# buaacyw/MeshAnything

Hardware: NVIDIA H100
Metric: face-tokens/sec (350M, 800-face cap) (higher is better)
Workload: dtype f16 weights/activations, f32 accumulate

## Files before the change

meshanything_b200/csrc/api.cu:

```cuda
#include <stdarg.h>
#include <stdlib.h>
#include <stdio.h>
#include <string.h>

#include <atomic>
#include <map>
#include <mutex>
#include <vector>

#include "canon.cuh"
#include "internal.h"

namespace ma {

static thread_local char g_err[512] = "";
static std::atomic<unsigned long long> g_launches{0};

void set_error(const char* fmt, ...) {
  va_list ap;
  va_start(ap, fmt);
  vsnprintf(g_err, sizeof(g_err), fmt, ap);
  va_end(ap);
}
void count_launch(int n) { g_launches += (unsigned long long)n; }
// ... 303 lines not shown
  if (!logits || !out_tokens || B < 1 || vocab < 1) {
    set_error("ma_sample_tokens: bad arguments");
    return 1;
  }
  SampleArgs sa;
  memset(&sa, 0, sizeof(sa));
  sa.logits = (const __half*)logits; sa.vocab = vocab; sa.B = B; sa.max_new = 1; sa.eos_id = -1; sa.pad_id = -1;
  sa.do_sample = sampling ? sampling->do_sample : 0;
  sa.top_k = sampling ? sampling->top_k : 0;
  sa.top_p = sampling ? sampling->top_p : 1.0f;
  sa.seed = sampling ? sampling->seed : 0;
  sa.first = 1; sa.token_out = out_tokens; sa.support_out = out_support;
  return launch_sample(sa, (cudaStream_t)stream);
}

size_t ma_kv_cache_bytes(int n_layers, int B, int tmax) {
  return (size_t)n_layers * 2 * B * NHEAD * (size_t)tmax * HD * sizeof(__half);
}

size_t ma_decoder_workspace_bytes(int B, int tmax) { return carve(nullptr, B, tmax, 8195 + 61).total; }

int ma_decode_generate(const ma_decoder_weights* w, const float* prefix, int B, int tmax, int max_new,
                       const ma_sampling* sampling, int eos_id, int pad_id, void* kv, void* ws_, int32_t* out_ids,
                       int32_t* out_lens, const int32_t* forced_ids, void* logits_out, int flags, void* stream) {
  if (!w || !prefix || !kv || !ws_ || !out_ids || B <= 0 || max_new <= 0) {
    set_error("ma_decode_generate: bad arguments");
    return 1;
  }
  if (check_decode_args("ma_decode_generate", w, B, tmax, max_new)) return 1;
  std::lock_guard<std::mutex> lock(g_mu);
  if (ensure_globals()) return 1;
  cudaStream_t user = (cudaStream_t)stream;
  cudaStream_t st = g_stream;
  cudaEventRecord(g_ev_in, user);
  cudaStreamWaitEvent(st, g_ev_in, 0);

  const long T = tmax;
  DecWs ws = carve(ws_, B, tmax, 8195 + 61);
  cudaMemsetAsync(ws.attn_scratch, 0, ws.attn_scratch_bytes, st);
  cudaMemsetAsync(ws.attn_scratch_pre, 0, ws.attn_scratch_pre_bytes, st);
  cudaMemsetAsync(ws.fast, 0, fast_workspace_bytes(), st);
  if (launch_fill_i32(out_ids, pad_id, (long)B * max_new, st)) return 1;

  SampleArgs sa;
  fill_sample_args(sa, w, ws, B, max_new, sampling, eos_id, pad_id, out_ids);
  sa.first = 1; sa.forced = forced_ids; sa.logits_out = (__half*)logits_out;
  sa.all_done = ws.all_done;

  const bool tc = use_tc(B, sa.do_sample, flags);
  if (tc) cudaMemsetAsync(ws.tc_scratch, 0, linear_ws_scratch_bytes(), st);
  const bool fast = (B == 1) && !(flags & MA_GEN_NO_FAST);
  bool mega = fast && !sa.do_sample && !(flags & MA_GEN_NO_MEGA) && mega_fits(tmax) && mega_supported();
  if (fast) sa.nkeys_next = fast_nkeys_ptr(ws.fast);
  if (mega && mega_prepare(w, ws.mega, st)) mega = false;

  for (int b0 = 0; b0 < B; b0 += PREFILL_SEQS) {
    const int nb = std::min(PREFILL_SEQS, B - b0), M = nb * PREFIX;
    if (launch_embed_prefix(w, prefix + (size_t)b0 * PREFIX * HID, nb, ws.hres, ws.x16, ws.nkeys, st)) return 1;
    if (run_layers(w, ws, kv, B, T, M, PREFIX, b0, PREFIX, st, tc)) return 1;
    if (launch_gather_rows(ws.x16, HID, PREFIX - 1, PREFIX, nb, ws.lastx16 + (size_t)b0 * HID, st)) return 1;
  }
  if (dec_linear(tc, ws, w->lm_head, nullptr, ws.lastx16, HID, ws.logits, w->vocab, B, w->vocab, HID, MA_EPI_NONE, st))
    return 1;
  if (launch_sample(sa, st)) return 1;
  sa.first = 0;
  sa.nkeys_next = nullptr;


  const bool use_graph = !(flags & MA_GEN_NO_GRAPH);
  const bool early = !(flags & MA_GEN_NO_EARLY_EXIT) && !forced_ids;
  const int CHECK_EVERY = 64;
  const unsigned long long whash = use_graph ? weights_hash(w) : 0;
  bool flag_pending = false;
  int rc = 0;
  if (mega) {
    const int MEGA_STEPS = 512;
    for (int i = 1; i < max_new && rc == 0; i += MEGA_STEPS) {
      rc = mega_enqueue(w, ws.s, tmax, (__half*)kv, ws.mega, sa, std::min(MEGA_STEPS, max_new - i), i - 1,
                        (flags & MA_GEN_TRACE) ? 1 : 0, st);
    }
  }
  for (int i = 1; i < max_new && rc == 0 && !mega; i++) {
    const int ctx = PREFIX + i;
    const int bucket = fast ? 0 : (ctx + 1023) / 1024;
    const int max_keys = fast ? tmax : std::min(tmax, bucket * 1024);
    auto enqueue = [&](cudaStream_t s) -> int {
      if (fast) return fast_step_enqueue(w, ws.s, tmax, (__half*)kv, ws.fast, sa, !(flags & MA_GEN_NO_PDL), s);
      return enqueue_batched_step(w, ws, kv, B, T, max_keys, sa, s, tc);
    };
    if (!use_graph) {
      rc = enqueue(st);
    } else {
      GraphKey key;
      memset(&key, 0, sizeof(key));
      key.w = w; key.kv = kv; key.ws = ws_; key.out_ids = out_ids; key.forced = forced_ids; key.logits_out = logits_out;
      key.B = B; key.tmax = tmax; key.max_new = max_new; key.bucket = bucket; key.flags = flags;
      key.do_sample = sa.do_sample; key.top_k = sa.top_k; key.eos = eos_id; key.pad = pad_id; key.top_p = sa.top_p;
      key.seed = sa.do_sample ? sa.seed : 0;
      key.whash = whash;
      key.ws_mode = linear_ws_mode();
      if (launch_cached_graph(key, st, enqueue)) return 1;
    }
    if (early && (i % CHECK_EVERY) == 0) {
      if (flag_pending && cudaEventQuery(g_ev_flag) == cudaSuccess) {
        if (*g_flag_host == 1) break;
        flag_pending = false;
      }
      if (!flag_pending) {
        cudaMemcpyAsync(g_flag_host, ws.all_done, sizeof(int), cudaMemcpyDeviceToHost, st);
        cudaEventRecord(g_ev_flag, st);
        flag_pending = true;
      }
    }
  }
  if (rc) return rc;
  if (out_lens) cudaMemcpyAsync(out_lens, ws.s.lens, sizeof(int) * B, cudaMemcpyDeviceToDevice, st);
  cudaEventRecord(g_ev_out, st);
  cudaStreamWaitEvent(user, g_ev_out, 0);
  return check_launch("ma_decode_generate") ? 0 : 1;
}



static int slots_enter(void* stream, cudaStream_t* st) {
  if (ensure_globals()) return 1;
  cudaEventRecord(g_ev_in, (cudaStream_t)stream);
  cudaStreamWaitEvent(g_stream, g_ev_in, 0);
  *st = g_stream;
  return 0;
}
static int slots_leave(void* stream, const char* who) {
  cudaEventRecord(g_ev_out, g_stream);
  cudaStreamWaitEvent((cudaStream_t)stream, g_ev_out, 0);
  return check_launch(who) ? 0 : 1;
}

int ma_decode_slots_init(int B, int tmax, int pad_id, void* ws_, void* stream) {
  if (!ws_ || B <= 0 || tmax < PREFIX + 1) {
    set_error("ma_decode_slots_init: bad arguments");
    return 1;
  }
  std::lock_guard<std::mutex> lock(g_mu);
  cudaStream_t st;
  if (slots_enter(stream, &st)) return 1;
  DecWs ws = carve(ws_, B, tmax, 8195 + 61);
  cudaMemsetAsync(ws.attn_scratch, 0, ws.attn_scratch_bytes, st);
  cudaMemsetAsync(ws.attn_scratch_pre, 0, ws.attn_scratch_pre_bytes, st);
  cudaMemsetAsync(ws.tc_scratch, 0, linear_ws_scratch_bytes(), st);
  if (launch_fill_i32(ws.s.pos, PREFIX, B, st) || launch_fill_i32(ws.s.gen, 0, B, st) ||
      launch_fill_i32(ws.s.tok, pad_id, B, st) || launch_fill_i32(ws.s.finished, 1, B, st) ||
      launch_fill_i32(ws.s.lens, 0, B, st) || launch_fill_i32(ws.s.sid, 0, B, st)) return 1;
  return slots_leave(stream, "ma_decode_slots_init");
}

int ma_decode_slot_stream(int slot, int B, int tmax, int stream_id, void* ws_, void* stream) {
  if (!ws_ || slot < 0 || slot >= B) {
    set_error("ma_decode_slot_stream: bad arguments (slot %d of %d)", slot, B);
    return 1;
  }
  std::lock_guard<std::mutex> lock(g_mu);
  cudaStream_t st;
  if (slots_enter(stream, &st)) return 1;
  DecWs ws = carve(ws_, B, tmax, 8195 + 61);
  if (launch_fill_i32(ws.s.sid + slot, stream_id, 1, st)) return 1;
  return slots_leave(stream, "ma_decode_slot_stream");
}

int ma_decode_slots_seek(int B, int tmax, int pos, int gen, int tok, void* ws_, void* stream) {
  if (!ws_ || B <= 0 || pos < PREFIX || pos >= tmax || gen < 1) {
    set_error("ma_decode_slots_seek: bad arguments (pos %d of tmax %d)", pos, tmax);
// ... 117 lines not shown
```

meshanything_b200/csrc/attention.cu:

```cuda
#include "canon.cuh"
#include "internal.h"

namespace ma {

constexpr int ATT_THREADS = 256;
constexpr int PART = 66;

struct AttnSmem {
  __half k[MA_ATTN_CHUNK * HD];
  __half v[MA_ATTN_CHUNK * HD];
  float s[MA_ATTN_CHUNK];
  float red[8][65];
  float wmax[8];
  uint64_t bar[2];
  int last;
};

struct AttnArgs {
  const __half* q;
  int ldq;
  const __half* K;
  const __half* V;
  long T;
  int H;
  int rows_per_slot;
  const int* slots;
  const int* nkeys;
  float scale;
  __half* out;
  int ldo;
  float* part;
  int* counters;
  int max_chunks;
  int decode_prefetch;
};

__global__ void __launch_bounds__(ATT_THREADS) attention_kernel(AttnArgs a) {
  extern __shared__ __align__(128) unsigned char smem_raw[];
  AttnSmem& sm = *reinterpret_cast<AttnSmem*>(smem_raw);
  const int c = blockIdx.x, h = blockIdx.y, m = blockIdx.z;
  const int tid = threadIdx.x, warp = tid >> 5, lane = tid & 31, grp = lane >> 3, li = lane & 7;

  if (!a.decode_prefetch) pdl_wait();
  const int n = min(a.nkeys[m], a.max_chunks * MA_ATTN_CHUNK);
  if (c * MA_ATTN_CHUNK >= n) return;
  const int len = min(MA_ATTN_CHUNK, n - c * MA_ATTN_CHUNK);
  const int nch = (n + MA_ATTN_CHUNK - 1) / MA_ATTN_CHUNK;
  const int slot = a.slots ? a.slots[m] : m / a.rows_per_slot;
  const long base = (((long)slot * a.H + h) * a.T + (long)c * MA_ATTN_CHUNK) * HD;

  const int len_early = a.decode_prefetch ? max(0, min(len, (n - 1) - c * MA_ATTN_CHUNK)) : 0;
  if (tid == 0) {
    mbar_init(&sm.bar[0], 1);
    mbar_init(&sm.bar[1], 1);
    mbar_fence_init();
    if (len_early > 0) {
      mbar_expect_tx(&sm.bar[0], 2u * len_early * HD * 2);
      bulk_g2s(sm.k, a.K + base, len_early * HD * 2, &sm.bar[0]);
      bulk_g2s(sm.v, a.V + base, len_early * HD * 2, &sm.bar[0]);
    }
  }
  if (a.decode_prefetch) pdl_wait();
  pdl_trigger();
  if (tid == 0) {
    const int rest = len - len_early;
    if (rest > 0) {
      mbar_expect_tx(&sm.bar[1], 2u * rest * HD * 2);
      bulk_g2s(sm.k + len_early * HD, a.K + base + (long)len_early * HD, rest * HD * 2, &sm.bar[1]);
      bulk_g2s(sm.v + len_early * HD, a.V + base + (long)len_early * HD, rest * HD * 2, &sm.bar[1]);
    }
  }
  float qf[8];
  {
    uint4 u = *reinterpret_cast<const uint4*>(a.q + (long)m * a.ldq + h * HD + 8 * li);
    unpack8(u, qf);
  }
  __syncthreads();
  if (len_early > 0) mbar_wait(&sm.bar[0], 0);
  if (len - len_early > 0) mbar_wait(&sm.bar[1], 0);

  float lmax = -INFINITY;
#pragma unroll
  for (int rho = 0; rho < MA_ATTN_CHUNK / 32; rho++) {
    const int r = 32 * rho + 4 * warp + grp;
    const int rr = min(r, len - 1);
    uint4 u = *reinterpret_cast<const uint4*>(sm.k + rr * HD + 8 * li);
    float kf[8];
    unpack8(u, kf);
    float p = 0.0f;
#pragma unroll
    for (int j = 0; j < 8; j++) p = ffma(qf[j], kf[j], p);
    p = fadd(p, __shfl_xor_sync(0xffffffffu, p, 4));
    p = fadd(p, __shfl_xor_sync(0xffffffffu, p, 2));
    p = fadd(p, __shfl_xor_sync(0xffffffffu, p, 1));
    const float s = fmul(p, a.scale);
    if (r < len) {
      if (li == 0) sm.s[r] = s;
      lmax = fmaxf(lmax, s);
    }
  }
  lmax = warp_max(lmax);
  if (lane == 0) sm.wmax[warp] = lmax;
  __syncthreads();
  float cmax = sm.wmax[0];
#pragma unroll
  for (int w = 1; w < 8; w++) cmax = fmaxf(cmax, sm.wmax[w]);

  float l = 0.0f, o[8];
#pragma unroll
  for (int j = 0; j < 8; j++) o[j] = 0.0f;
#pragma unroll
  for (int rho = 0; rho < MA_ATTN_CHUNK / 32; rho++) {
    const int r = 32 * rho + 4 * warp + grp;
    if (r < len) {
      const float e = ma_exp(fsub(sm.s[r], cmax));
      l = fadd(l, e);
      uint4 u = *reinterpret_cast<const uint4*>(sm.v + r * HD + 8 * li);
      const float pf = __half2float(__float2half_rn(e));
      float vf[8];
      unpack8(u, vf);
#pragma unroll
      for (int j = 0; j < 8; j++) o[j] = ffma(pf, vf[j], o[j]);
    }
  }
  l = fadd(l, __shfl_xor_sync(0xffffffffu, l, 16));
  l = fadd(l, __shfl_xor_sync(0xffffffffu, l, 8));
#pragma unroll
  for (int j = 0; j < 8; j++) {
    o[j] = fadd(o[j], __shfl_xor_sync(0xffffffffu, o[j], 16));
    o[j] = fadd(o[j], __shfl_xor_sync(0xffffffffu, o[j], 8));
  }
  if (grp == 0) {
#pragma unroll
    for (int j = 0; j < 8; j++) sm.red[warp][8 * li + j] = o[j];
    if (li == 0) sm.red[warp][64] = l;
  }
  __syncthreads();
  float* part = a.part + (((long)m * a.H + h) * a.max_chunks) * PART;
  if (tid < 65) {
    float x[8];
#pragma unroll
    for (int w = 0; w < 8; w++) x[w] = sm.red[w][tid];
    const float r = fadd(fadd(fadd(x[0], x[1]), fadd(x[2], x[3])), fadd(fadd(x[4], x[5]), fadd(x[6], x[7])));
    if (nch == 1) {
      sm.red[0][tid] = r;
    } else {
      part[c * PART + (tid < 64 ? tid : 65)] = r;
      if (tid == 64) part[c * PART + 64] = cmax;
    }
  }
  if (nch > 1) {
    __threadfence();
    __syncthreads();
    if (tid == 0) {
      int* cnt = a.counters + (long)m * a.H + h;
      const int prev = atomicAdd(cnt, 1);
      sm.last = (prev == nch - 1);
      if (sm.last) *cnt = 0;
    }
    __syncthreads();
    if (!sm.last) return;
    __threadfence();
    if (tid < 64) {
      float M = -INFINITY;
      for (int cc = 0; cc < nch; cc++) M = fmaxf(M, __ldcg(part + cc * PART + 64));
      float L = 0.0f, O = 0.0f;
      for (int cc = 0; cc < nch; cc++) {
        const float w = ma_exp(fsub(__ldcg(part + cc * PART + 64), M));
        L = ffma(__ldcg(part + cc * PART + 65), w, L);
        O = ffma(__ldcg(part + cc * PART + tid), w, O);
      }
      a.out[(long)m * a.ldo + h * HD + tid] = __float2half_rn(__fdiv_rn(O, L));
    }
  } else {
    __syncthreads();
    if (tid < 64) {
      const float L = sm.red[0][64], O = sm.red[0][tid];
      a.out[(long)m * a.ldo + h * HD + tid] = __float2half_rn(__fdiv_rn(O, L));
    }
  }
}

size_t attention_scratch_bytes(int M, int H, int max_keys) {
  const size_t chunks = (size_t)(max_keys + MA_ATTN_CHUNK - 1) / MA_ATTN_CHUNK;
  return (size_t)M * H * chunks * PART * sizeof(float) + (size_t)M * H * sizeof(int) + 256;
}

int launch_attention_ex(const __half* q, int ldq, const __half* K, const __half* V, long T, int H, int rows_per_slot,
                        const int* slots, const int* nkeys, int max_keys, int M, float scale, __half* out, int ldo,
                        void* scratch, int decode_prefetch, bool pdl, cudaStream_t st) {
  if (M <= 0) return 0;
  static bool attr_done = false;
  if (!attr_done) {
    cudaFuncSetAttribute(attention_kernel, cudaFuncAttributeMaxDynamicSharedMemorySize, (int)sizeof(AttnSmem));
    attr_done = true;
  }
  const int chunks = (max_keys + MA_ATTN_CHUNK - 1) / MA_ATTN_CHUNK;
  AttnArgs a;
  a.q = q; a.ldq = ldq; a.K = K; a.V = V; a.T = T; a.H = H;
  a.rows_per_slot = rows_per_slot > 0 ? rows_per_slot : 1;
  a.slots = slots; a.nkeys = nkeys; a.scale = scale; a.out = out; a.ldo = ldo;
  a.counters = reinterpret_cast<int*>(scratch);
  size_t coff = ((size_t)M * H * sizeof(int) + 255) & ~(size_t)255;
  a.part = reinterpret_cast<float*>(reinterpret_cast<char*>(scratch) + coff);
  a.max_chunks = chunks;
  a.decode_prefetch = decode_prefetch;
  dim3 grid(chunks, H, M);
  cudaLaunchConfig_t cfg = {};
  cfg.gridDim = grid;
  cfg.blockDim = dim3(ATT_THREADS);
  cfg.dynamicSmemBytes = sizeof(AttnSmem);
  cfg.stream = st;
  cudaLaunchAttribute at[1];
  at[0].id = cudaLaunchAttributeProgrammaticStreamSerialization;
  at[0].val.programmaticStreamSerializationAllowed = 1;
  cfg.attrs = at;
  cfg.numAttrs = pdl ? 1 : 0;
  cudaLaunchKernelEx(&cfg, attention_kernel, a);
  count_launch();
  return check_launch("attention_kernel") ? 0 : 1;
}

int launch_attention(const __half* q, int ldq, const __half* K, const __half* V, long T, int H, int rows_per_slot,
                     const int* slots, const int* nkeys, int max_keys, int M, float scale, __half* out, int ldo,
                     void* scratch, cudaStream_t st) {
  return launch_attention_ex(q, ldq, K, V, T, H, rows_per_slot, slots, nkeys, max_keys, M, scale, out, ldo, scratch, 0,
                             false, st);
}

}
```

meshanything_b200/csrc/canon.cuh:

```cuda
#pragma once
#include <cuda_fp16.h>
#include <cuda_runtime.h>
#include <stdint.h>

#include "../../include/ma_canon_constants.h"

namespace ma {

__device__ __forceinline__ float fadd(float a, float b) { return __fadd_rn(a, b); }
__device__ __forceinline__ float fsub(float a, float b) { return __fsub_rn(a, b); }
__device__ __forceinline__ float fmul(float a, float b) { return __fmul_rn(a, b); }
__device__ __forceinline__ float ffma(float a, float b, float c) { return __fmaf_rn(a, b, c); }

__device__ __forceinline__ float ma_exp(float x) {
  if (x < MA_EXP_FLUSH) return 0.0f;
  float y = fmul(x, MA_LOG2E);
  float n = rintf(y);
  float f = fsub(y, n);
  float p = MA_EXP2_C6;
  p = ffma(p, f, MA_EXP2_C5);
  p = ffma(p, f, MA_EXP2_C4);
  p = ffma(p, f, MA_EXP2_C3);
  p = ffma(p, f, MA_EXP2_C2);
  p = ffma(p, f, MA_EXP2_C1);
// ... 61 lines not shown
  }
  return v[0];
}

template <int ORD>
__device__ __forceinline__ float transpose_reduce32o(float* v, int lane) {
#pragma unroll
  for (int k = 0; k < 5; k++) {
    const int s = 16 >> k;
    const int m = ORD ? (k == 0 ? 4 : k == 1 ? 2 : k == 2 ? 1 : k == 3 ? 8 : 16) : s;
    const bool up = (lane & m) != 0;
#pragma unroll
    for (int i = 0; i < s; i++) {
      float mine = up ? v[i + s] : v[i];
      float other = up ? v[i] : v[i + s];
      float recv = __shfl_xor_sync(0xffffffffu, other, m);
      v[i] = fadd(mine, recv);
    }
  }
  return v[0];
}
template <int ORD>
__device__ __forceinline__ int transpose_owner(int lane) {
  if (!ORD) return lane;
  return ((lane & 4) ? 16 : 0) | ((lane & 2) ? 8 : 0) | ((lane & 1) ? 4 : 0) | ((lane & 8) ? 2 : 0) | ((lane & 16) ? 1 : 0);
}
__device__ __forceinline__ float warp_sum_seg64(float v) {
  v = fadd(v, __shfl_xor_sync(0xffffffffu, v, 4));
  v = fadd(v, __shfl_xor_sync(0xffffffffu, v, 2));
  v = fadd(v, __shfl_xor_sync(0xffffffffu, v, 1));
  v = fadd(v, __shfl_xor_sync(0xffffffffu, v, 8));
  v = fadd(v, __shfl_xor_sync(0xffffffffu, v, 16));
  return v;
}
__device__ __forceinline__ float tree16_push(float v, int g, float* lv) {
  if (g & 1) {
    v = fadd(lv[0], v);
    if (g & 2) {
      v = fadd(lv[1], v);
      if (g & 4) {
        v = fadd(lv[2], v);
        if (g & 8) v = fadd(lv[3], v); else lv[3] = v;
      } else lv[2] = v;
    } else lv[1] = v;
  } else lv[0] = v;
  return v;
}
__device__ __forceinline__ float tree4_push(float v, int g, float* lv) {
  if (g == 0) lv[0] = v;
  else if (g == 1) lv[0] = fadd(lv[0], v);
  else if (g == 2) lv[1] = v;
  else v = fadd(lv[0], fadd(lv[1], v));
  return v;
}

__device__ __forceinline__ float warp_tree(const float* s, int n) {
  float b[8];
#pragma unroll
  for (int i = 0; i < 8; i++) b[i] = (i < n) ? s[i] : 0.0f;
  if (n == 8) return fadd(fadd(fadd(b[0], b[1]), fadd(b[2], b[3])), fadd(fadd(b[4], b[5]), fadd(b[6], b[7])));
  if (n == 6) return fadd(fadd(fadd(b[0], b[1]), fadd(b[2], b[3])), fadd(b[4], b[5]));
  if (n == 4) return fadd(fadd(b[0], b[1]), fadd(b[2], b[3]));
  if (n == 2) return fadd(b[0], b[1]);
  int m = n;
  while (m > 1) {
    int k = 0;
    for (int i = 0; i + 1 < m; i += 2) b[k++] = fadd(b[i], b[i + 1]);
    if (m & 1) b[k++] = b[m - 1];
    m = k;
  }
  return b[0];
}

__device__ __forceinline__ float block_sum4(float x0, float x1, float x2, float x3, float* red) {
  float p = fadd(fadd(x0, x1), fadd(x2, x3));
  p = warp_sum(p);
  const int nw = blockDim.x >> 5;
  __syncthreads();
  if ((threadIdx.x & 31) == 0) red[threadIdx.x >> 5] = p;
  __syncthreads();
  return warp_tree(red, nw);
}

__device__ __forceinline__ void layernorm4(float* x, const float* __restrict__ gamma, const float* __restrict__ beta,
                                           float eps, int W, float* red) {
  const float inv = __fdiv_rn(1.0f, (float)W);
  float mean = fmul(block_sum4(x[0], x[1], x[2], x[3], red), inv);
  float d0 = fsub(x[0], mean), d1 = fsub(x[1], mean), d2 = fsub(x[2], mean), d3 = fsub(x[3], mean);
  float var = fmul(block_sum4(fmul(d0, d0), fmul(d1, d1), fmul(d2, d2), fmul(d3, d3), red), inv);
  float rstd = __fdiv_rn(1.0f, __fsqrt_rn(fadd(var, eps)));
  const float4 g = *reinterpret_cast<const float4*>(gamma + 4 * threadIdx.x);
  const float4 b = *reinterpret_cast<const float4*>(beta + 4 * threadIdx.x);
  x[0] = ffma(fmul(d0, rstd), g.x, b.x);
  x[1] = ffma(fmul(d1, rstd), g.y, b.y);
  x[2] = ffma(fmul(d2, rstd), g.z, b.z);
  x[3] = ffma(fmul(d3, rstd), g.w, b.w);
}

__device__ __forceinline__ uint32_t smem_u32(const void* p) { return (uint32_t)__cvta_generic_to_shared(p); }
__device__ __forceinline__ void mbar_init(uint64_t* bar, uint32_t count) {
  asm volatile("mbarrier.init.shared::cta.b64 [%0], %1;" ::"r"(smem_u32(bar)), "r"(count));
}
__device__ __forceinline__ void mbar_fence_init() { asm volatile("fence.mbarrier_init.release.cluster;" ::: "memory"); }
__device__ __forceinline__ void mbar_expect_tx(uint64_t* bar, uint32_t bytes) {
  asm volatile("mbarrier.arrive.expect_tx.shared::cta.b64 _, [%0], %1;" ::"r"(smem_u32(bar)), "r"(bytes) : "memory");
}
__device__ __forceinline__ void mbar_wait(uint64_t* bar, uint32_t parity) {
  asm volatile(
      "{\n\t.reg .pred p;\n\t"
      "WAIT_%=:\n\t"
      "mbarrier.try_wait.parity.shared::cta.b64 p, [%0], %1;\n\t"
      "@p bra DONE_%=;\n\t"
      "bra WAIT_%=;\n\t"
      "DONE_%=:\n\t}" ::"r"(smem_u32(bar)),
      "r"(parity)
      : "memory");
}
__device__ __forceinline__ void bulk_g2s(void* dst, const void* src, uint32_t bytes, uint64_t* bar) {
  asm volatile("cp.async.bulk.shared::cluster.global.mbarrier::complete_tx::bytes [%0], [%1], %2, [%3];" ::"r"(
                   smem_u32(dst)),
               "l"(src), "r"(bytes), "r"(smem_u32(bar))
               : "memory");
}

__device__ __forceinline__ void pdl_trigger() { asm volatile("griddepcontrol.launch_dependents;" ::: "memory"); }
__device__ __forceinline__ void pdl_wait() { asm volatile("griddepcontrol.wait;" ::: "memory"); }

}
```

meshanything_b200/csrc/decode_fast.cu:

```cuda
#include "canon.cuh"
#include "internal.h"

namespace ma {

int launch_attention_ex(const __half* q, int ldq, const __half* K, const __half* V, long T, int H, int rows_per_slot,
                        const int* slots, const int* nkeys, int max_keys, int M, float scale, __half* out, int ldo,
                        void* scratch, int decode_prefetch, bool pdl, cudaStream_t st);

constexpr int FG_THREADS = 256;
constexpr int FG_WARPS = 8;

enum { MODE_QKV = 0, MODE_OUT = 1, MODE_FC1 = 2, MODE_FC2 = 3, MODE_LM = 4 };

struct FastWs {
  float hresA[HID];
  float hresB[HID];
  __half q[HID];
  __half attn16[HID];
  __half y16[HID];
  __half f16[FFN];
  __half logits[8256];
  float cand_val[256];
  int cand_idx[256];
  int counter;
  int nkeys;
  alignas(256) unsigned char attn_scratch[256];
};

struct FastArgs {
  const __half* W;
  const __half* bias;
  int N, rows_per_cta;
  const float* hres_in;
  const __half* y16_in;
  const float *gamma, *beta;
  const __half* x16_in;
  float* hres_out;
  int embed;
  const float *extra, *tok_pos, *cond, *pos_table;
  const __half* tok_table;
  SeqState s;
  __half* out16;
  __half *kc, *vc;
  long T;
  FastWs* ws;
  int do_argmax;
  int max_new, eos_id, pad_id;
  int32_t* out_ids;
  const int32_t* forced;
  __half* logits_out;
  int* all_done;
  int vocab;
};

template <int K>
struct alignas(128) FastSmemHdr {
  uint64_t bar[FG_WARPS];
  float red[8];
  float bval[FG_WARPS];
  int bidx[FG_WARPS];
  int last;
  alignas(16) __half xs[K];
};

template <int K, int MODE>
__global__ void __launch_bounds__(FG_THREADS) fast_gemv_kernel(FastArgs a) {
  extern __shared__ __align__(128) unsigned char smem_raw[];
  FastSmemHdr<K>& sh = *reinterpret_cast<FastSmemHdr<K>*>(smem_raw);
  __half* sw = reinterpret_cast<__half*>(smem_raw + sizeof(FastSmemHdr<K>));
  const int tid = threadIdx.x, warp = tid >> 5, lane = tid & 31;

  if (MODE != MODE_QKV) pdl_trigger();

  const int row0 = blockIdx.x * a.rows_per_cta;
  const int nrows = max(0, min(a.rows_per_cta, a.N - row0));
  const int base = nrows / FG_WARPS, rem = nrows % FG_WARPS;
  const int wr0 = warp * base + min(warp, rem);
  const int wn = base + (warp < rem ? 1 : 0);

  if (lane == 0) {
    mbar_init(&sh.bar[warp], 1);
    mbar_fence_init();
  }
  __syncwarp();
  if (lane == 0 && wn > 0) {
    mbar_expect_tx(&sh.bar[warp], (uint32_t)wn * K * 2);
    bulk_g2s(sw + (size_t)wr0 * K, a.W + (size_t)(row0 + wr0) * K, (uint32_t)wn * K * 2, &sh.bar[warp]);
  }

  pdl_wait();
  if (MODE == MODE_QKV) pdl_trigger();

  if (MODE == MODE_QKV || MODE == MODE_FC1 || MODE == MODE_LM) {
    float v[4];
    if (MODE == MODE_QKV && a.embed) {
      const int tok = a.s.tok[0], gen = a.s.gen[0], pos = a.s.pos[0];
      float4 X;
      int fidx;
      if (tok < 3) {
        X = *reinterpret_cast<const float4*>(a.extra + (long)tok * HID + 4 * tid);
        fidx = tok;
      } else {
        const uint2 u = *reinterpret_cast<const uint2*>(a.tok_table + (long)(tok - 3) * HID + 4 * tid);
        const __half2* h = reinterpret_cast<const __half2*>(&u);
        const float2 p0 = __half22float2(h[0]), p1 = __half22float2(h[1]);
        X = make_float4(p0.x, p0.y, p1.x, p1.y);
        int r = (gen - 2) % 9;
        if (r < 0) r += 9;
        fidx = r + 3;
      }
      const float4 F = *reinterpret_cast<const float4*>(a.tok_pos + (long)fidx * HID + 4 * tid);
      const float4 C = *reinterpret_cast<const float4*>(a.cond + HID + 4 * tid);
      const float4 P = *reinterpret_cast<const float4*>(a.pos_table + (long)(pos + 2) * HID + 4 * tid);
      v[0] = fadd(fadd(fadd(X.x, F.x), C.x), P.x);
      v[1] = fadd(fadd(fadd(X.y, F.y), C.y), P.y);
      v[2] = fadd(fadd(fadd(X.z, F.z), C.z), P.z);
      v[3] = fadd(fadd(fadd(X.w, F.w), C.w), P.w);
    } else {
      const float4 hv = *reinterpret_cast<const float4*>(a.hres_in + 4 * tid);
      const uint2 u = *reinterpret_cast<const uint2*>(a.y16_in + 4 * tid);
      const __half2* h = reinterpret_cast<const __half2*>(&u);
      const float2 p0 = __half22float2(h[0]), p1 = __half22float2(h[1]);
      v[0] = fadd(hv.x, p0.x); v[1] = fadd(hv.y, p0.y); v[2] = fadd(hv.z, p1.x); v[3] = fadd(hv.w, p1.y);
      layernorm4(v, a.gamma, a.beta, MA_LN_EPS, HID, sh.red);
    }
    if (blockIdx.x == 0 && a.hres_out)
      *reinterpret_cast<float4*>(a.hres_out + 4 * tid) = make_float4(v[0], v[1], v[2], v[3]);
    __half2 h0 = __floats2half2_rn(v[0], v[1]), h1 = __floats2half2_rn(v[2], v[3]);
    uint2 u;
    u.x = *reinterpret_cast<uint32_t*>(&h0);
    u.y = *reinterpret_cast<uint32_t*>(&h1);
    *reinterpret_cast<uint2*>(sh.xs + 4 * tid) = u;
  } else {
    for (int i = tid; i < K / 8; i += FG_THREADS)
      *reinterpret_cast<uint4*>(sh.xs + 8 * i) = *reinterpret_cast<const uint4*>(a.x16_in + 8 * i);
  }
  __syncthreads();

  constexpr int G = K / 256;
  uint4 xp[G];
#pragma unroll
  for (int g = 0; g < G; g++) xp[g] = *reinterpret_cast<const uint4*>(sh.xs + 256 * g + 8 * lane);

  int pos = 0;
  if (MODE == MODE_QKV) pos = a.s.pos[0];
  float bestv = -INFINITY;
  int besti = 0x7fffffff;

  if (wn > 0) mbar_wait(&sh.bar[warp], 0);
  constexpr int RB = (K == HID) ? 4 : 1;
  for (int r0 = 0; r0 < wn; r0 += RB) {
    float acc[RB];
#pragma unroll
    for (int i = 0; i < RB; i++) acc[i] = 0.0f;
#pragma unroll
    for (int g = 0; g < G; g++) {
      float xf[8];
      unpack8(xp[g], xf);
#pragma unroll
      for (int i = 0; i < RB; i++) {
        const int r = min(r0 + i, wn - 1);
        const uint4 u = *reinterpret_cast<const uint4*>(sw + (size_t)(wr0 + r) * K + 256 * g + 8 * lane);
        float wf[8];
        unpack8(u, wf);
#pragma unroll
        for (int j = 0; j < 8; j++) acc[i] = ffma(wf[j], xf[j], acc[i]);
      }
    }
#pragma unroll
    for (int i = 0; i < RB; i++) {
      const float sum = warp_sum(acc[i]);
      const int n = row0 + wr0 + r0 + i;
      if (r0 + i < wn && lane == 0) {
        const float bf = a.bias ? __half2float(a.bias[n]) : 0.0f;
        __half h = __float2half_rn(fadd(sum, bf));
        if (MODE == MODE_FC1 && __half2float(h) < 0.0f) h = __float2half_rn(0.0f);
        if (MODE == MODE_QKV) {
          if (n < HID) {
            a.out16[n] = h;
          } else {
            const int e = (n - HID) & (HID - 1), head = e >> 6, d = e & 63;
            __half* c = (n < 2 * HID) ? a.kc : a.vc;
            c[((long)head * a.T + pos) * HD + d] = h;
          }
        } else {
          a.out16[n] = h;
        }
        if (MODE == MODE_LM) {
          const float v = __half2float(h);
          if (v > bestv || (v == bestv && n < besti)) { bestv = v; besti = n; }
        }
      }
    }
  }

  if (MODE == MODE_LM) {
    FastWs* ws = a.ws;
    const int gen = a.s.gen[0];
    if (a.logits_out) {
      __syncthreads();
      for (int i = tid; i < nrows; i += FG_THREADS)
        a.logits_out[(long)gen * a.vocab + row0 + i] = a.out16[row0 + i];
    }
    if (!a.do_argmax) return;
    if (lane == 0) { sh.bval[warp] = bestv; sh.bidx[warp] = besti; }
    __syncthreads();
    if (tid == 0) {
      float bv = sh.bval[0];
      int bi = sh.bidx[0];
      for (int w = 1; w < FG_WARPS; w++)
        if (sh.bval[w] > bv || (sh.bval[w] == bv && sh.bidx[w] < bi)) { bv = sh.bval[w]; bi = sh.bidx[w]; }
      ws->cand_val[blockIdx.x] = bv;
      ws->cand_idx[blockIdx.x] = bi;
      __threadfence();
      const int prev = atomicAdd(&ws->counter, 1);
      sh.last = (prev == (int)gridDim.x - 1);
      if (sh.last) ws->counter = 0;
    }
    __syncthreads();
    if (!sh.last) return;
    __threadfence();
    float bv = -INFINITY;
    int bi = 0x7fffffff;
    for (int i = tid; i < (int)gridDim.x; i += FG_THREADS) {
      const float v = __ldcg(&ws->cand_val[i]);
      const int ix = __ldcg(&ws->cand_idx[i]);
      if (v > bv || (v == bv && ix < bi)) { bv = v; bi = ix; }
    }
#pragma unroll
    for (int o = 16; o > 0; o >>= 1) {
      const float ov = __shfl_xor_sync(0xffffffffu, bv, o);
      const int oi = __shfl_xor_sync(0xffffffffu, bi, o);
      if (ov > bv || (ov == bv && oi < bi)) { bv = ov; bi = oi; }
    }
    if (lane == 0) { sh.bval[warp] = bv; sh.bidx[warp] = bi; }
    __syncthreads();
    if (tid == 0) {
      for (int w = 1; w < FG_WARPS; w++)
        if (sh.bval[w] > bv || (sh.bval[w] == bv && sh.bidx[w] < bi)) { bv = sh.bval[w]; bi = sh.bidx[w]; }
      int tok = bi;
      if (a.forced) tok = a.forced[gen];
      int fin = a.s.finished[0];
      if (fin) tok = a.pad_id;
      if (gen < a.max_new) a.out_ids[gen] = tok;
      if (!fin) a.s.lens[0] = gen + 1;
      if (!fin && tok == a.eos_id) fin = 1;
      a.s.finished[0] = fin;
      a.s.tok[0] = tok;
      a.s.gen[0] = gen + 1;
      const int np = a.s.pos[0] + 1;
      a.s.pos[0] = np;
      ws->nkeys = np + 1;
      if (a.all_done) *a.all_done = fin;
    }
  }
}

static int g_sms = 0;

size_t fast_workspace_bytes() {
  return sizeof(FastWs) + attention_scratch_bytes(1, NHEAD, 18432) + 256;
}

template <int K, int MODE>
static int launch_fast(const FastArgs& a, int grid, bool pdl, cudaStream_t st) {
  const size_t smem = sizeof(FastSmemHdr<K>) + (size_t)a.rows_per_cta * K * 2;
  static size_t attr_set = 0;
  if (smem > attr_set) {
    cudaFuncSetAttribute(fast_gemv_kernel<K, MODE>, cudaFuncAttributeMaxDynamicSharedMemorySize, (int)smem);
    attr_set = smem;
  }
  cudaLaunchConfig_t cfg = {};
  cfg.gridDim = dim3(grid);
  cfg.blockDim = dim3(FG_THREADS);
  cfg.dynamicSmemBytes = smem;
  cfg.stream = st;
  cudaLaunchAttribute at[1];
  at[0].id = cudaLaunchAttributeProgrammaticStreamSerialization;
  at[0].val.programmaticStreamSerializationAllowed = 1;
  cfg.attrs = at;
  cfg.numAttrs = pdl ? 1 : 0;
  cudaLaunchKernelEx(&cfg, fast_gemv_kernel<K, MODE>, a);
  count_launch();
  return check_launch("fast_gemv_kernel") ? 0 : 1;
}

int fast_step_enqueue(const ma_decoder_weights* w, SeqState s, int tmax, __half* kv, void* fast_ws,
                      const SampleArgs& sa, bool pdl, cudaStream_t st) {
  if (!g_sms) {
    int dev = 0;
    cudaGetDevice(&dev);
    cudaDeviceGetAttribute(&g_sms, cudaDevAttrMultiProcessorCount, dev);
    if (g_sms <= 0 || g_sms > 256) g_sms = 132;
  }
  const int grid = g_sms;
  FastWs* ws = reinterpret_cast<FastWs*>(fast_ws);
  const long T = tmax;
  auto rpc = [&](int N) { return (N + grid - 1) / grid; };

  FastArgs base;
  memset(&base, 0, sizeof(base));
  base.s = s;
  base.T = T;
  base.ws = ws;
  base.extra = w->extra; base.tok_pos = w->tok_pos; base.cond = w->cond; base.pos_table = w->pos;
  base.tok_table = (const __half*)w->tok_table;
  base.vocab = w->vocab;

  for (int L = 0; L < w->n_layers; L++) {
    __half* kc = kv + ((size_t)(L * 2 + 0)) * NHEAD * T * HD;
    __half* vc = kv + ((size_t)(L * 2 + 1)) * NHEAD * T * HD;
    {
      FastArgs a = base;
      a.W = (const __half*)w->wqkv[L]; a.bias = (const __half*)w->bqkv[L]; a.N = QKV; a.rows_per_cta = rpc(QKV);
      a.embed = (L == 0);
      if (L > 0) { a.hres_in = ws->hresB; a.y16_in = ws->y16; a.gamma = w->ln2g[L - 1]; a.beta = w->ln2b[L - 1]; }
      a.hres_out = ws->hresA;
      a.out16 = ws->q; a.kc = kc; a.vc = vc;
      if (launch_fast<HID, MODE_QKV>(a, grid, pdl, st)) return 1;
    }
    if (launch_attention_ex(ws->q, HID, kc, vc, T, NHEAD, 1, nullptr, &ws->nkeys, tmax, 1, 0.125f, ws->attn16, HID,
                            ws->attn_scratch, 1, pdl, st)) return 1;
    {
      FastArgs a = base;
      a.W = (const __half*)w->wo[L]; a.bias = (const __half*)w->bo[L]; a.N = HID; a.rows_per_cta = rpc(HID);
      a.x16_in = ws->attn16; a.out16 = ws->y16;
      if (launch_fast<HID, MODE_OUT>(a, grid, pdl, st)) return 1;
    }
    {
      FastArgs a = base;
      a.W = (const __half*)w->w1[L]; a.bias = (const __half*)w->b1[L]; a.N = FFN; a.rows_per_cta = rpc(FFN);
      a.hres_in = ws->hresA; a.y16_in = ws->y16; a.gamma = w->ln1g[L]; a.beta = w->ln1b[L];
      a.hres_out = ws->hresB; a.out16 = ws->f16;
      if (launch_fast<HID, MODE_FC1>(a, grid, pdl, st)) return 1;
    }
    {
      FastArgs a = base;
      a.W = (const __half*)w->w2[L]; a.bias = (const __half*)w->b2[L]; a.N = HID; a.rows_per_cta = rpc(HID);
      a.x16_in = ws->f16; a.out16 = ws->y16;
      if (launch_fast<FFN, MODE_FC2>(a, grid, pdl, st)) return 1;
    }
  }
  {
    FastArgs a = base;
    const int L = w->n_layers - 1;
    a.W = (const __half*)w->lm_head; a.bias = nullptr; a.N = w->vocab; a.rows_per_cta = rpc(w->vocab);
    a.hres_in = ws->hresB; a.y16_in = ws->y16; a.gamma = w->ln2g[L]; a.beta = w->ln2b[L];
    a.out16 = sa.do_sample ? const_cast<__half*>(sa.logits) : ws->logits;
    a.do_argmax = !sa.do_sample;
    a.max_new = sa.max_new; a.eos_id = sa.eos_id; a.pad_id = sa.pad_id;
    a.out_ids = sa.out_ids; a.forced = sa.forced; a.logits_out = sa.logits_out; a.all_done = sa.all_done;
    if (launch_fast<HID, MODE_LM>(a, grid, pdl, st)) return 1;
  }
  if (sa.do_sample) {
    SampleArgs s2 = sa;
    s2.logits_out = nullptr;
    s2.nkeys_next = &ws->nkeys;
    if (launch_sample(s2, st)) return 1;
  }
  return 0;
}

int* fast_nkeys_ptr(void* fast_ws) { return &reinterpret_cast<FastWs*>(fast_ws)->nkeys; }

}
```

meshanything_b200/csrc/elementwise.cu:

```cuda
#include "canon.cuh"
#include "internal.h"

namespace ma {

__global__ void layernorm_kernel(const float* __restrict__ x, const __half* __restrict__ res16,
                                 const float* __restrict__ gamma, const float* __restrict__ beta, float eps, int W,
                                 float* __restrict__ out32, __half* __restrict__ out16) {
  __shared__ float red[8];
  const long row = blockIdx.x;
  const int t = threadIdx.x;
  pdl_trigger();
  pdl_wait();
  float v[4];
  if (x) {
    const float4 xv = *reinterpret_cast<const float4*>(x + row * W + 4 * t);
    v[0] = xv.x; v[1] = xv.y; v[2] = xv.z; v[3] = xv.w;
  } else {
    v[0] = v[1] = v[2] = v[3] = 0.0f;
  }
  if (res16) {
    const uint2 u = *reinterpret_cast<const uint2*>(res16 + row * W + 4 * t);
    const __half2* h = reinterpret_cast<const __half2*>(&u);
    const float2 a = __half22float2(h[0]), b = __half22float2(h[1]);
    if (x) {
      v[0] = fadd(v[0], a.x); v[1] = fadd(v[1], a.y); v[2] = fadd(v[2], b.x); v[3] = fadd(v[3], b.y);
    } else {
      v[0] = a.x; v[1] = a.y; v[2] = b.x; v[3] = b.y;
    }
  }
  layernorm4(v, gamma, beta, eps, W, red);
  if (out32) *reinterpret_cast<float4*>(out32 + row * W + 4 * t) = make_float4(v[0], v[1], v[2], v[3]);
  if (out16) {
    __half2 h0 = __floats2half2_rn(v[0], v[1]), h1 = __floats2half2_rn(v[2], v[3]);
    uint2 u;
    u.x = *reinterpret_cast<uint32_t*>(&h0);
    u.y = *reinterpret_cast<uint32_t*>(&h1);
    *reinterpret_cast<uint2*>(out16 + row * W + 4 * t) = u;
  }
}

int launch_layernorm(const float* x, const __half* res16, const float* gamma, const float* beta, float eps, int M,
                     int W, float* out32, __half* out16, cudaStream_t st, bool pdl) {
  if (M <= 0) return 0;
  if (W % 128 != 0 || W > 1024 || (!x && !res16)) {
    set_error("ma_layernorm: unsupported width %d or no input", W);
    return 1;
  }
  cudaLaunchConfig_t cfg = {};
  cfg.gridDim = dim3(M);
  cfg.blockDim = dim3(W / 4);
  cfg.stream = st;
  cudaLaunchAttribute at[1];
  at[0].id = cudaLaunchAttributeProgrammaticStreamSerialization;
  at[0].val.programmaticStreamSerializationAllowed = 1;
  cfg.attrs = at;
  cfg.numAttrs = pdl ? 1 : 0;
  cudaLaunchKernelEx(&cfg, layernorm_kernel, x, res16, gamma, beta, eps, W, out32, out16);
  count_launch();
  return check_launch("layernorm_kernel") ? 0 : 1;
}

__device__ __forceinline__ void store_row4(float* hres, __half* x16, long row, int t, const float* v) {
  *reinterpret_cast<float4*>(hres + row * HID + 4 * t) = make_float4(v[0], v[1], v[2], v[3]);
  __half2 h0 = __floats2half2_rn(v[0], v[1]), h1 = __floats2half2_rn(v[2], v[3]);
  uint2 u;
  u.x = *reinterpret_cast<uint32_t*>(&h0);
  u.y = *reinterpret_cast<uint32_t*>(&h1);
  *reinterpret_cast<uint2*>(x16 + row * HID + 4 * t) = u;
}

__global__ void embed_prefix_kernel(const float* __restrict__ prefix, const float* __restrict__ cond,
                                    const float* __restrict__ pos, float* __restrict__ hres, __half* __restrict__ x16,
                                    int* __restrict__ nkeys) {
  const long row = blockIdx.x;
  const int s = (int)(row % PREFIX), t = threadIdx.x;
  const float4 p = *reinterpret_cast<const float4*>(prefix + row * HID + 4 * t);
  const float4 c = *reinterpret_cast<const float4*>(cond + 4 * t);
  const float4 e = *reinterpret_cast<const float4*>(pos + (long)(s + 2) * HID + 4 * t);
  float v[4] = {fadd(fadd(p.x, c.x), e.x), fadd(fadd(p.y, c.y), e.y), fadd(fadd(p.z, c.z), e.z),
                fadd(fadd(p.w, c.w), e.w)};
  store_row4(hres, x16, row, t, v);
  if (t == 0) nkeys[row] = s + 1;
}

int launch_embed_prefix(const ma_decoder_weights* w, const float* prefix, int B, float* hres, __half* x16, int* nkeys,
                        cudaStream_t st) {
  embed_prefix_kernel<<<B * PREFIX, HID / 4, 0, st>>>(prefix, w->cond, w->pos, hres, x16, nkeys);
  count_launch();
  return check_launch("embed_prefix_kernel") ? 0 : 1;
}

__device__ __forceinline__ void token_embedding4(const ma_decoder_weights& w, int tok, int gen, int pos, int t,
                                                 float* v) {
  float4 X;
  int fidx;
  if (tok < 3) {
    X = *reinterpret_cast<const float4*>(w.extra + (long)tok * HID + 4 * t);
    fidx = tok;
  } else {
    const uint2 u = *reinterpret_cast<const uint2*>(reinterpret_cast<const __half*>(w.tok_table) +
                                                    (long)(tok - 3) * HID + 4 * t);
    const __half2* h = reinterpret_cast<const __half2*>(&u);
    const float2 a = __half22float2(h[0]), b = __half22float2(h[1]);
    X = make_float4(a.x, a.y, b.x, b.y);
    int r = (gen - 2) % 9;
    if (r < 0) r += 9;
    fidx = r + 3;
  }
  const float4 F = *reinterpret_cast<const float4*>(w.tok_pos + (long)fidx * HID + 4 * t);
  const float4 C = *reinterpret_cast<const float4*>(w.cond + HID + 4 * t);
  const float4 P = *reinterpret_cast<const float4*>(w.pos + (long)(pos + 2) * HID + 4 * t);
  v[0] = fadd(fadd(fadd(X.x, F.x), C.x), P.x);
  v[1] = fadd(fadd(fadd(X.y, F.y), C.y), P.y);
// ... 273 lines not shown
```

meshanything_b200/csrc/internal.h:

```cpp
#pragma once
#include <cuda_fp16.h>
#include <cuda_runtime.h>
#include <stdint.h>

#include "../../include/meshanything_b200.h"

namespace ma {

constexpr int HID = 1024;
constexpr int NHEAD = 16;
constexpr int HD = 64;
constexpr int FFN = 4096;
constexpr int PREFIX = 257;
constexpr int QKV = 3 * HID;

struct SeqState {
  int* pos;
  int* gen;
  int* tok;
  int* finished;
  int* lens;
  int* sid;
};

void set_error(const char* fmt, ...);
void count_launch(int n = 1);
bool check_launch(const char* what);

int launch_linear(const __half* W, const __half* bias, const __half* x, int ldx, __half* y, int ldy, int M, int N,
                  int K, int epi, cudaStream_t st);

bool attention_tc_supported(int ldq, int ldo, long T, long Tpad, int nkeys, const void* q, const void* K, const void* Vt,
                            const void* out);
int launch_attention_tc(const __half* q, int ldq, const __half* K, const __half* Vt, long T, long Tpad, int H,
                        int rows_per_slot, int n_slots, int nkeys, float scale, __half* out, int ldo, cudaStream_t st);
int launch_scatter_heads_t(const __half* src, int ld, int col0, int head_stride, int H, int n, long Tpad, int n_slots,
                           __half* dst, cudaStream_t st);

bool linear_tc_supported(int M, int N, int K, int ldx, int ldy, const void* x, const void* W, const void* y);
int launch_linear_tc(const __half* W, const __half* bias, const __half* x, int ldx, __half* y, int ldy, int M, int N,
                     int K, int epi, cudaStream_t st);

size_t linear_ws_scratch_bytes();
void linear_ws_set_mode(int cluster);
int linear_ws_mode();
bool linear_ws_supported(int M, int N, int K, int ldx, const void* x, const void* W);
int launch_linear_ws(const __half* W, const __half* bias, const __half* x, int ldx, __half* y, int ldy, int M, int N,
                     int K, int epi, void* scratch, cudaStream_t st, bool pdl = false);

size_t attention_scratch_bytes(int M, int H, int max_keys);
int launch_attention_decode(const __half* qkv, int ldq, __half* K, __half* V, long T, const int* nkeys, int max_keys,
                            int M, float scale, __half* out, int ldo, void* scratch, bool pdl, cudaStream_t st);
int launch_attention(const __half* q, int ldq, const __half* K, const __half* V, long T, int H, int rows_per_slot,
                     const int* slots, const int* nkeys, int max_keys, int M, float scale, __half* out, int ldo,
                     void* scratch, cudaStream_t st);

int launch_layernorm(const float* x, const __half* res16, const float* gamma, const float* beta, float eps, int M,
                     int W, float* out32, __half* out16, cudaStream_t st, bool pdl = false);
int launch_embed_prefix(const ma_decoder_weights* w, const float* prefix, int B, float* hres, __half* x16, int* nkeys,
                        cudaStream_t st);
int launch_embed_tokens(const ma_decoder_weights* w, SeqState s, int B, float* hres, __half* x16, int* nkeys,
                        cudaStream_t st);
int launch_kv_append(const __half* qkv, int M, int rows_per_slot, const int* nkeys, __half* kc, __half* vc, long T,
                     cudaStream_t st);
int launch_gather_rows(const __half* src, int ld, int row0, int stride, int B, __half* dst, cudaStream_t st);
struct SampleArgs {
  const __half* logits;
  int vocab, B, max_new, eos_id, pad_id;
  int do_sample, top_k;
  float top_p;
  unsigned long long seed;
  SeqState s;
  int first;
  int32_t* out_ids;
  const int32_t* forced;
  __half* logits_out;
  int* all_done;
  int* nkeys_next;
  int32_t* support_out;
  int32_t* token_out;
  int row0, nrows;
  int slots;
};
int launch_sample(const SampleArgs& a, cudaStream_t st);
int launch_fill_i32(int32_t* p, int v, long n, cudaStream_t st);

int* fast_nkeys_ptr(void* fast_ws);
size_t fast_workspace_bytes();
int fast_step_enqueue(const ma_decoder_weights* w, SeqState s, int tmax, __half* kv, void* fast_ws,
                      const SampleArgs& sa, bool pdl, cudaStream_t st);


size_t mega_workspace_bytes();
int mega_prepare(const ma_decoder_weights* w, void* mega_ws, cudaStream_t st);
int mega_enqueue(const ma_decoder_weights* w, SeqState s, int tmax, __half* kv, void* mega_ws, const SampleArgs& sa,
                 int n_steps, int step_base, int trace, cudaStream_t st);
int mega_supported();
bool mega_fits(int tmax);
void mega_set_debug(unsigned long long timeout_ns, int fault);
int mega_error_flag_offset();
int mega_trace_offset();
int mega_trace_cta_offset();

}
```

Measured before the change: 1321.

## Bucket fast-path attention keys, stage merge partials and bias/LN params early

```diff
diff --git a/meshanything_b200/csrc/api.cu b/meshanything_b200/csrc/api.cu
--- a/meshanything_b200/csrc/api.cu
+++ b/meshanything_b200/csrc/api.cu
@@ -409,10 +409,11 @@
   }
   for (int i = 1; i < max_new && rc == 0 && !mega; i++) {
     const int ctx = PREFIX + i;
-    const int bucket = fast ? 0 : (ctx + 1023) / 1024;
-    const int max_keys = fast ? tmax : std::min(tmax, bucket * 1024);
+    const int bucket = (ctx + 1023) / 1024;
+    const int max_keys = std::min(tmax, bucket * 1024);
     auto enqueue = [&](cudaStream_t s) -> int {
-      if (fast) return fast_step_enqueue(w, ws.s, tmax, (__half*)kv, ws.fast, sa, !(flags & MA_GEN_NO_PDL), s);
+      if (fast)
+        return fast_step_enqueue(w, ws.s, tmax, max_keys, (__half*)kv, ws.fast, sa, !(flags & MA_GEN_NO_PDL), s);
       return enqueue_batched_step(w, ws, kv, B, T, max_keys, sa, s, tc);
     };
     if (!use_graph) {
diff --git a/meshanything_b200/csrc/attention.cu b/meshanything_b200/csrc/attention.cu
--- a/meshanything_b200/csrc/attention.cu
+++ b/meshanything_b200/csrc/attention.cu
@@ -5,6 +5,7 @@
 
 constexpr int ATT_THREADS = 256;
 constexpr int PART = 66;
+constexpr int ATT_MERGE_BLOCK = 2 * MA_ATTN_CHUNK * HD * 2 / (PART * 4);
 
 struct AttnSmem {
   __half k[MA_ATTN_CHUNK * HD];
@@ -161,17 +162,27 @@
     __syncthreads();
     if (!sm.last) return;
     __threadfence();
-    if (tid < 64) {
-      float M = -INFINITY;
+    float* pst = reinterpret_cast<float*>(sm.k);
+    const bool single = nch <= ATT_MERGE_BLOCK;
+    float M = -INFINITY, L = 0.0f, O = 0.0f;
+    if (!single && tid < 64)
       for (int cc = 0; cc < nch; cc++) M = fmaxf(M, __ldcg(part + cc * PART + 64));
-      float L = 0.0f, O = 0.0f;
-      for (int cc = 0; cc < nch; cc++) {
-        const float w = ma_exp(fsub(__ldcg(part + cc * PART + 64), M));
-        L = ffma(__ldcg(part + cc * PART + 65), w, L);
-        O = ffma(__ldcg(part + cc * PART + tid), w, O);
+    for (int c0 = 0; c0 < nch; c0 += ATT_MERGE_BLOCK) {
+      const int nb = min(ATT_MERGE_BLOCK, nch - c0);
+      for (int t = tid; t < nb * PART; t += ATT_THREADS) pst[t] = __ldcg(part + (long)c0 * PART + t);
+      __syncthreads();
+      if (tid < 64) {
+        if (single)
+          for (int cc = 0; cc < nb; cc++) M = fmaxf(M, pst[cc * PART + 64]);
+        for (int cc = 0; cc < nb; cc++) {
+          const float w = ma_exp(fsub(pst[cc * PART + 64], M));
+          L = ffma(pst[cc * PART + 65], w, L);
+          O = ffma(pst[cc * PART + tid], w, O);
+        }
       }
-      a.out[(long)m * a.ldo + h * HD + tid] = __float2half_rn(__fdiv_rn(O, L));
-    }
+      __syncthreads();
+    }
+    if (tid < 64) a.out[(long)m * a.ldo + h * HD + tid] = __float2half_rn(__fdiv_rn(O, L));
   } else {
     __syncthreads();
     if (tid < 64) {
diff --git a/meshanything_b200/csrc/canon.cuh b/meshanything_b200/csrc/canon.cuh
--- a/meshanything_b200/csrc/canon.cuh
+++ b/meshanything_b200/csrc/canon.cuh
@@ -167,15 +167,12 @@
   return warp_tree(red, nw);
 }
 
-__device__ __forceinline__ void layernorm4(float* x, const float* __restrict__ gamma, const float* __restrict__ beta,
-                                           float eps, int W, float* red) {
+__device__ __forceinline__ void layernorm4(float* x, const float4& g, const float4& b, float eps, int W, float* red) {
   const float inv = __fdiv_rn(1.0f, (float)W);
   float mean = fmul(block_sum4(x[0], x[1], x[2], x[3], red), inv);
   float d0 = fsub(x[0], mean), d1 = fsub(x[1], mean), d2 = fsub(x[2], mean), d3 = fsub(x[3], mean);
   float var = fmul(block_sum4(fmul(d0, d0), fmul(d1, d1), fmul(d2, d2), fmul(d3, d3), red), inv);
   float rstd = __fdiv_rn(1.0f, __fsqrt_rn(fadd(var, eps)));
-  const float4 g = *reinterpret_cast<const float4*>(gamma + 4 * threadIdx.x);
-  const float4 b = *reinterpret_cast<const float4*>(beta + 4 * threadIdx.x);
   x[0] = ffma(fmul(d0, rstd), g.x, b.x);
   x[1] = ffma(fmul(d1, rstd), g.y, b.y);
   x[2] = ffma(fmul(d2, rstd), g.z, b.z);
diff --git a/meshanything_b200/csrc/decode_fast.cu b/meshanything_b200/csrc/decode_fast.cu
--- a/meshanything_b200/csrc/decode_fast.cu
+++ b/meshanything_b200/csrc/decode_fast.cu
@@ -68,6 +68,7 @@
   extern __shared__ __align__(128) unsigned char smem_raw[];
   FastSmemHdr<K>& sh = *reinterpret_cast<FastSmemHdr<K>*>(smem_raw);
   __half* sw = reinterpret_cast<__half*>(smem_raw + sizeof(FastSmemHdr<K>));
+  __half* sb = sw + (size_t)a.rows_per_cta * K;
   const int tid = threadIdx.x, warp = tid >> 5, lane = tid & 31;
 
   if (MODE != MODE_QKV) pdl_trigger();
@@ -86,6 +87,15 @@
   if (lane == 0 && wn > 0) {
     mbar_expect_tx(&sh.bar[warp], (uint32_t)wn * K * 2);
     bulk_g2s(sw + (size_t)wr0 * K, a.W + (size_t)(row0 + wr0) * K, (uint32_t)wn * K * 2, &sh.bar[warp]);
+  }
+  if (a.bias)
+    for (int i = tid; i < nrows; i += FG_THREADS) sb[i] = a.bias[row0 + i];
+  float4 ln_g, ln_b, cond;
+  if (MODE == MODE_QKV && a.embed) {
+    cond = *reinterpret_cast<const float4*>(a.cond + HID + 4 * tid);
+  } else if (MODE == MODE_QKV || MODE == MODE_FC1 || MODE == MODE_LM) {
+    ln_g = *reinterpret_cast<const float4*>(a.gamma + 4 * tid);
+    ln_b = *reinterpret_cast<const float4*>(a.beta + 4 * tid);
   }
 
   pdl_wait();
@@ -110,7 +120,7 @@
         fidx = r + 3;
       }
       const float4 F = *reinterpret_cast<const float4*>(a.tok_pos + (long)fidx * HID + 4 * tid);
-      const float4 C = *reinterpret_cast<const float4*>(a.cond + HID + 4 * tid);
+      const float4 C = cond;
       const float4 P = *reinterpret_cast<const float4*>(a.pos_table + (long)(pos + 2) * HID + 4 * tid);
       v[0] = fadd(fadd(fadd(X.x, F.x), C.x), P.x);
       v[1] = fadd(fadd(fadd(X.y, F.y), C.y), P.y);
@@ -122,7 +132,7 @@
       const __half2* h = reinterpret_cast<const __half2*>(&u);
       const float2 p0 = __half22float2(h[0]), p1 = __half22float2(h[1]);
       v[0] = fadd(hv.x, p0.x); v[1] = fadd(hv.y, p0.y); v[2] = fadd(hv.z, p1.x); v[3] = fadd(hv.w, p1.y);
-      layernorm4(v, a.gamma, a.beta, MA_LN_EPS, HID, sh.red);
+      layernorm4(v, ln_g, ln_b, MA_LN_EPS, HID, sh.red);
     }
     if (blockIdx.x == 0 && a.hres_out)
       *reinterpret_cast<float4*>(a.hres_out + 4 * tid) = make_float4(v[0], v[1], v[2], v[3]);
@@ -172,7 +182,7 @@
       const float sum = warp_sum(acc[i]);
       const int n = row0 + wr0 + r0 + i;
       if (r0 + i < wn && lane == 0) {
-        const float bf = a.bias ? __half2float(a.bias[n]) : 0.0f;
+        const float bf = a.bias ? __half2float(sb[wr0 + r0 + i]) : 0.0f;
         __half h = __float2half_rn(fadd(sum, bf));
         if (MODE == MODE_FC1 && __half2float(h) < 0.0f) h = __float2half_rn(0.0f);
         if (MODE == MODE_QKV) {
@@ -264,7 +274,7 @@
 
 template <int K, int MODE>
 static int launch_fast(const FastArgs& a, int grid, bool pdl, cudaStream_t st) {
-  const size_t smem = sizeof(FastSmemHdr<K>) + (size_t)a.rows_per_cta * K * 2;
+  const size_t smem = sizeof(FastSmemHdr<K>) + (size_t)a.rows_per_cta * K * 2 + (((size_t)a.rows_per_cta * 2 + 15) & ~(size_t)15);
   static size_t attr_set = 0;
   if (smem > attr_set) {
     cudaFuncSetAttribute(fast_gemv_kernel<K, MODE>, cudaFuncAttributeMaxDynamicSharedMemorySize, (int)smem);
@@ -285,7 +295,7 @@
   return check_launch("fast_gemv_kernel") ? 0 : 1;
 }
 
-int fast_step_enqueue(const ma_decoder_weights* w, SeqState s, int tmax, __half* kv, void* fast_ws,
+int fast_step_enqueue(const ma_decoder_weights* w, SeqState s, int tmax, int max_keys, __half* kv, void* fast_ws,
                       const SampleArgs& sa, bool pdl, cudaStream_t st) {
   if (!g_sms) {
     int dev = 0;
@@ -319,7 +329,7 @@
       a.out16 = ws->q; a.kc = kc; a.vc = vc;
       if (launch_fast<HID, MODE_QKV>(a, grid, pdl, st)) return 1;
     }
-    if (launch_attention_ex(ws->q, HID, kc, vc, T, NHEAD, 1, nullptr, &ws->nkeys, tmax, 1, 0.125f, ws->attn16, HID,
+    if (launch_attention_ex(ws->q, HID, kc, vc, T, NHEAD, 1, nullptr, &ws->nkeys, max_keys, 1, 0.125f, ws->attn16, HID,
                             ws->attn_scratch, 1, pdl, st)) return 1;
     {
       FastArgs a = base;
diff --git a/meshanything_b200/csrc/elementwise.cu b/meshanything_b200/csrc/elementwise.cu
--- a/meshanything_b200/csrc/elementwise.cu
+++ b/meshanything_b200/csrc/elementwise.cu
@@ -28,7 +28,8 @@
       v[0] = a.x; v[1] = a.y; v[2] = b.x; v[3] = b.y;
     }
   }
-  layernorm4(v, gamma, beta, eps, W, red);
+  layernorm4(v, *reinterpret_cast<const float4*>(gamma + 4 * t), *reinterpret_cast<const float4*>(beta + 4 * t), eps, W,
+             red);
   if (out32) *reinterpret_cast<float4*>(out32 + row * W + 4 * t) = make_float4(v[0], v[1], v[2], v[3]);
   if (out16) {
     __half2 h0 = __floats2half2_rn(v[0], v[1]), h1 = __floats2half2_rn(v[2], v[3]);
diff --git a/meshanything_b200/csrc/internal.h b/meshanything_b200/csrc/internal.h
--- a/meshanything_b200/csrc/internal.h
+++ b/meshanything_b200/csrc/internal.h
@@ -87,7 +87,7 @@
 
 int* fast_nkeys_ptr(void* fast_ws);
 size_t fast_workspace_bytes();
-int fast_step_enqueue(const ma_decoder_weights* w, SeqState s, int tmax, __half* kv, void* fast_ws,
+int fast_step_enqueue(const ma_decoder_weights* w, SeqState s, int tmax, int max_keys, __half* kv, void* fast_ws,
                       const SampleArgs& sa, bool pdl, cudaStream_t st);
 
 
```

Result: faster. 1464, median of 6 (+10.8%).
